# baler-collaboration/baler

Hardware: AMD Instinct MI355X
Metric: rows/sec (train) + rows/sec (encode), CMS 24-col AE at 1/2/4/8 GPUs (higher is better)
Workload: dtype f32

## Files before the change

baler_amd/csrc/fused.hip:

```cpp
#include "fused.hpp"

#include <cmath>
#include <cstdlib>
#include <type_traits>
#include <utility>

namespace bamd {
namespace {

using v4 = float __attribute__((ext_vector_type(4)));

__host__ __device__ constexpr int tiles(int d) { return (d + 15) / 16; }
__host__ __device__ constexpr int tile_steps(int d, int t) {
    return d - 16 * t >= 16 ? 4 : (d - 16 * t + 3) / 4;
}
__host__ __device__ constexpr int slot_feature(int d, int t, int g, int r) {
    int v = d - 16 * t;
    if (v >= 16) return 16 * t + 4 * g + r;
    return 4 * r + g < v ? 16 * t + 4 * r + g : -1;
}

constexpr int kQS = 68;
constexpr int kRowsPerWG = 64;

// ... 2094 lines not shown
        const bool v0 = r0 < n, v1 = r1 < n;
        constexpr int es = DZ16 ? 2 : 4;
        const __amdgpu_buffer_rsrc_t xrs = __builtin_amdgcn_make_buffer_rsrc((void *)((const char *)dz7 + (size_t)(grp * 128) * F * es), 0,
                                                                             0x7fffffff, 0x00020000);
        const int lr0 = wave * 32 + (lane & 15);
        const int xo0 = ((v0 ? lr0 : 0) * F + 8 * g) * es, xo1 = ((v1 ? lr0 + 16 : 0) * F + 8 * g) * es;
        asm volatile("" : "+v"(ws.voff), "+v"(w7.voff));
        v4 d6a[13], d6b[13];
        zero_tiles(d6a);
        zero_tiles(d6b);
        wide_in_product_bf16<F, DZ16>(d6a, d6b, wst, w7, xrs, xo0, xo1, wave, lane, g);
        auto narrow = [&](v4 (&d6)[13], int64_t row, bool valid) {
            const int64_t rrow = valid ? row : 0;
            Ring ring;
            ring_prime<S::total>(ring, ws);
            {
                v4 a[13];
                load_act<200>(a, y7, rrow, g);
                lrelu_bwd(d6, a);
            }
            store_rows<200>(d6, dz6, 0, row, valid, lane, nullptr, nullptr);
            v4 d5[7], d4[4], d3[tiles(Z)], d2[4], d1[7], d0[13];
            bwd_layer<N, S, 6>(d6, d5, ring, ws);
            { v4 a[7]; load_act<100>(a, y6, rrow, g); lrelu_bwd(d5, a); }
            store_rows<100>(d5, dz5, 0, row, valid, lane, nullptr, nullptr);
            bwd_layer<N, S, 5>(d5, d4, ring, ws);
            { v4 a[4]; load_act<50>(a, y5, rrow, g); lrelu_bwd(d4, a); }
            store_rows<50>(d4, dz4, 0, row, valid, lane, nullptr, nullptr);
            bwd_layer<N, S, 4>(d4, d3, ring, ws);
            if (dz_latent) {
                v4 e[tiles(Z)];
                load_act<Z>(e, dz_latent, rrow, g);
#pragma unroll
                for (int t = 0; t < tiles(Z); ++t) d3[t] += e[t];
            }
            store_rows<Z>(d3, dz3, 0, row, valid, lane, nullptr, nullptr);
            bwd_layer<N, S, 3>(d3, d2, ring, ws);
            { v4 a[4]; load_act<50>(a, y3, rrow, g); lrelu_bwd(d2, a); }
            store_rows<50>(d2, dz2, 0, row, valid, lane, nullptr, nullptr);
            bwd_layer<N, S, 2>(d2, d1, ring, ws);
            { v4 a[7]; load_act<100>(a, y2, rrow, g); lrelu_bwd(d1, a); }
            store_rows<100>(d1, dz1, 0, row, valid, lane, nullptr, nullptr);
            bwd_layer<N, S, 1>(d1, d0, ring, ws);
            { v4 a[13]; load_act<200>(a, y1, rrow, g); lrelu_bwd(d0, a); }
            store_rows<200>(d0, dz0, 0, row, valid, lane, nullptr, nullptr);
        };
        narrow(d6a, r0, v0);
        narrow(d6b, r1, v1);
    }
}

template <int NT>
__device__ __forceinline__ void q_write(float *__restrict__ q, const v4 (&a)[NT], int lane, int wave) {
    typedef float __attribute__((address_space(3))) *lds_f;
    const int col = 16 * wave + (lane & 15), g = lane >> 4;
#pragma unroll
    for (int r = 0; r < 4; ++r) {
        lds_f p = (lds_f)q + ((4 * g + r) * kQS + col);
        asm volatile("" : "+v"(p));
#pragma unroll
        for (int t = 0; t < NT; ++t) p[t * 16 * kQS] = a[t][r];
    }
}
template <int D>
__device__ __forceinline__ void q_write_x(float *__restrict__ q, const v4 (&a)[tiles(D)], int lane, int wave) {
    static_assert(D % 16 != 0, "ones slot lives in the partial last tile");
    constexpr int T = tiles(D) - 1, V = D - 16 * T;
    constexpr int R1 = V / 4, G1 = V % 4;
    typedef float __attribute__((address_space(3))) *lds_f;
    const int col = 16 * wave + (lane & 15), g = lane >> 4;
#pragma unroll
    for (int r = 0; r < 4; ++r) {
        lds_f p = (lds_f)q + ((4 * g + r) * kQS + col);
        asm volatile("" : "+v"(p));
#pragma unroll
        for (int t = 0; t < tiles(D); ++t) {
            float v = a[t][r];
            if (t == T && r == R1 && g == G1) v = 1.0f;
            p[t * 16 * kQS] = v;
        }
    }
}

template <class N, int l> struct DW {
    static constexpr int NT = tiles(N::dim(l + 1)), KT = tiles(N::dim(l) + 1), TOT = NT * KT, T = (TOT + 3) / 4;
    static constexpr int rows_x = 16 * KT, rows_dz = 16 * NT;
};

template <class N, int l>
__device__ __forceinline__ void dw_phase(const float *__restrict__ qdz, const float *__restrict__ qx,
                                         v4 (&acc)[DW<N, l>::T], int lane, int wave) {
    using D = DW<N, l>;
    constexpr int NP = (D::T + 1) / 2, U = 4 * NP;
    const int g = lane >> 4, i = lane & 15;
    typedef const float __attribute__((address_space(3))) *lds_cf;
    typedef const v4 __attribute__((address_space(3))) *lds_cv4;
    const lds_cf la = (lds_cf)qdz + (i * kQS + 4 * g), lb = (lds_cf)qx + (i * kQS + 4 * g);
    const lds_cf la_w = la + wave * (16 * kQS);
    v4 fa[2][2], fb[2][2];
    auto lds_frags = [&](int u, v4 (&a)[2], v4 (&b)[2]) {
#pragma unroll
        for (int h = 0; h < 2; ++h) {
            const int it = 2 * (u >> 2) + h;
            if (it < D::T) {
                const int c = (4 * it) % D::NT, k0 = (4 * it) / D::NT;
                if (c + 3 < D::NT && 4 * it + 3 < D::TOT) {
                    a[h] = *(lds_cv4)(la_w + c * (16 * kQS) + 16 * (u & 3));
                    b[h] = *(lds_cv4)(lb + k0 * (16 * kQS) + 16 * (u & 3));
                } else {
                    int idx = wave + 4 * it;
                    idx = idx < D::TOT ? idx : D::TOT - 1;
                    const int kt = idx / D::NT, nt = idx - kt * D::NT;
                    a[h] = *(lds_cv4)(la + nt * (16 * kQS) + 16 * (u & 3));
                    b[h] = *(lds_cv4)(lb + kt * (16 * kQS) + 16 * (u & 3));
                }
            }
        }
    };
    lds_frags(0, fa[0], fb[0]);
#pragma unroll
    for (int u = 0; u < U; ++u) {
        if (u + 1 < U) lds_frags(u + 1, fa[(u + 1) & 1], fb[(u + 1) & 1]);
        __builtin_amdgcn_sched_barrier(0);
        const int it0 = 2 * (u >> 2), it1 = it0 + 1;
#pragma unroll
        for (int r = 0; r < 4; ++r) {
            acc[it0] = mfma(fa[u & 1][0][r], fb[u & 1][0][r], acc[it0]);
            if (it1 < D::T) acc[it1] = mfma(fa[u & 1][1][r], fb[u & 1][1][r], acc[it1]);
        }
        __builtin_amdgcn_sched_barrier(0);
    }
}

template <class N, int l>
__device__ __forceinline__ void dw_flush(v4 *__restrict__ slab, const v4 (&acc)[DW<N, l>::T], int lane, int wave) {
#pragma unroll
    for (int it = 0; it < DW<N, l>::T; ++it) {
        const int idx = wave + 4 * it;
        if (idx < DW<N, l>::TOT) slab[(int64_t)(N::slab_off(l) + idx) * gridDim.x * 64 + lane] = acc[it];
    }
}

constexpr int kImgB = 320;
template <class N> constexpr int img_a_rows();
template <class N> constexpr bool train_bias_in_lds() {
    return (size_t)(img_a_rows<N>() + kImgB) * kQS * sizeof(float) + (size_t)(N::bf_off(8) - N::bf_off(0)) * 16 <= 160 * 1024;
}
template <class N> constexpr int img_a_rows() {
    int m = 240;
    const int need[] = {DW<N, 7>::rows_x + DW<N, 7>::rows_dz, DW<N, 5>::rows_x + DW<N, 5>::rows_dz, DW<N, 2>::rows_x + DW<N, 2>::rows_dz,
                        DW<N, 0>::rows_x + DW<N, 0>::rows_dz};
    for (int v : need) m = v > m ? v : m;
    return m;
}

template <int F, int Z, bool RT = false>
__global__ void __launch_bounds__(256) train_dec_kernel(const v4 *packed, const void *__restrict__ xin, int in_f64,
                                                        int64_t n, const double *__restrict__ feats, v4 *__restrict__ slabs,
                                                        v4 *__restrict__ dz_out, int fr, int zr) {
    using N = Net<F, Z>;
    using S = StreamTrainDec<N>;
    constexpr int kImgA = img_a_rows<N>();
    static_assert(DW<N, 7>::rows_x + DW<N, 7>::rows_dz <= kImgA && DW<N, 6>::rows_x + DW<N, 6>::rows_dz <= kImgB &&
                  DW<N, 5>::rows_x + DW<N, 5>::rows_dz <= kImgA && DW<N, 4>::rows_x + DW<N, 4>::rows_dz <= kImgB, "image buffers");
    extern __shared__ __attribute__((aligned(16))) float lds[];
    float *imgA = lds, *imgB = lds + kImgA * kQS;
// ... 165 lines not shown

        q_write_x<F>(imgA, a0, lane, wave); q_write(imgA + DW<N, 0>::rows_x * kQS, d1, lane, wave);
        __syncthreads();
        dw_phase<N, 0>(imgA + DW<N, 0>::rows_x * kQS, imgA, g0, lane, wave);
        ring_tail<S::total>(ring, ws);
    }
    dw_flush<N, 1>(slab, g1, lane, wave); dw_flush<N, 0>(slab, g0, lane, wave);
}
#else
template <int F, int Z, bool RT = false>
__global__ void __launch_bounds__(256) train_enc_kernel(const v4 *packed, const void *__restrict__ xin, int in_f64,
                                                        int64_t n, const double *__restrict__ feats, v4 *__restrict__ slabs,
                                                        const v4 *__restrict__ dz_in, int fr, int zr) {
    using N = Net<F, Z>;
    using S = StreamTrainEnc<N>;
    static_assert(Z <= 16, "dL/dz hand-off is one tile per row");
    constexpr int kImgA = img_a_rows<N>();
    static_assert(DW<N, 3>::rows_x + DW<N, 3>::rows_dz <= kImgB && DW<N, 2>::rows_x + DW<N, 2>::rows_dz <= kImgA &&
                  DW<N, 1>::rows_x + DW<N, 1>::rows_dz <= kImgB && DW<N, 0>::rows_x + DW<N, 0>::rows_dz <= kImgA, "image buffers");
    extern __shared__ __attribute__((aligned(16))) float lds[];
    float *imgA = lds, *imgB = lds + kImgA * kQS;
    const v4 *bias_lds = packed + N::bf_off(0);
    if constexpr (train_bias_in_lds<N>()) {
        v4 *stage = (v4 *)(lds + (kImgA + kImgB) * kQS);
        stage_bias<N>(stage, packed);
        bias_lds = stage;
    }
    int lane = threadIdx.x & 63, wave = __builtin_amdgcn_readfirstlane(threadIdx.x >> 6);
    v4 *slab = slabs + (int64_t)blockIdx.x * 64;
    const int64_t ngroups = (n + kRowsPerWG - 1) / kRowsPerWG;
    WStream ws = make_stream(packed + S::start_f4, (N::packed_f4() - S::start_f4) * 16, threadIdx.x & 63);
    v4 g3[DW<N, 3>::T], g2[DW<N, 2>::T], g1[DW<N, 1>::T], g0[DW<N, 0>::T];
    zero_tiles(g3); zero_tiles(g2); zero_tiles(g1); zero_tiles(g0);
    Ring ring;
    ring_prime<S::total>(ring, ws);
    v4 a0n[tiles(F)], d4n;
    {
        const int64_t row0 = (int64_t)blockIdx.x * kRowsPerWG + 16 * wave + (lane & 15);
        load_rows<F, RT>(a0n, xin, in_f64, row0, row0 < n, lane, feats, fr);
        d4n = row0 < n ? dz_in[row0 * 4 + (lane >> 4)] : (v4){0.f, 0.f, 0.f, 0.f};
    }
    for (int64_t grp = blockIdx.x; grp < ngroups; grp += gridDim.x) {
        asm volatile("" : "+v"(ws.voff), "+s"(wave), "+v"(lane));
        const int64_t row = grp * kRowsPerWG + 16 * wave + (lane & 15);
        const int64_t row_next = row + (int64_t)gridDim.x * kRowsPerWG;
        const bool valid_next = row_next < n;
        RawRows<F> xraw;
        v4 a0[tiles(F)], a1[13], a2[7], a3[4], d4[tiles(Z)];
#pragma unroll
        for (int t = 0; t < tiles(F); ++t) a0[t] = a0n[t];
        d4[0] = d4n;
        fwd_layer<N, S, 0>(a0, a1, ring, ws, bias_lds, lane);
        fwd_layer<N, S, 1>(a1, a2, ring, ws, bias_lds, lane);
        fwd_layer<N, S, 2>(a2, a3, ring, ws, bias_lds, lane);
        v4 d3[4], d2[7], d1[13];
        q_write_x<50>(imgB, a3, lane, wave); q_write(imgB + DW<N, 3>::rows_x * kQS, d4, lane, wave);
        bwd_layer<N, S, 3>(d4, d3, ring, ws); lrelu_bwd(d3, a3);
        __syncthreads();
        dw_phase<N, 3>(imgB + DW<N, 3>::rows_x * kQS, imgB, g3, lane, wave);

        q_write_x<100>(imgA, a2, lane, wave); q_write(imgA + DW<N, 2>::rows_x * kQS, d3, lane, wave);
        bwd_layer<N, S, 2>(d3, d2, ring, ws); lrelu_bwd(d2, a2);
        __syncthreads();
        dw_phase<N, 2>(imgA + DW<N, 2>::rows_x * kQS, imgA, g2, lane, wave);

        q_write_x<200>(imgB, a1, lane, wave); q_write(imgB + DW<N, 1>::rows_x * kQS, d2, lane, wave);
        bwd_layer<N, S, 1>(d2, d1, ring, ws); lrelu_bwd(d1, a1);
        __syncthreads();
        load_rows_issue<F, RT>(xraw, xin, in_f64, row_next, valid_next, lane, fr);
        v4 dzraw = valid_next ? dz_in[row_next * 4 + (lane >> 4)] : (v4){0.f, 0.f, 0.f, 0.f};
        dw_phase<N, 1>(imgB + DW<N, 1>::rows_x * kQS, imgB, g1, lane, wave);
        load_rows_finish<F, RT>(a0n, xraw, valid_next, lane, feats, fr);
        d4n = dzraw;

        q_write_x<F>(imgA, a0, lane, wave); q_write(imgA + DW<N, 0>::rows_x * kQS, d1, lane, wave);
        __syncthreads();
        dw_phase<N, 0>(imgA + DW<N, 0>::rows_x * kQS, imgA, g0, lane, wave);
        ring_tail<S::total>(ring, ws);
    }
    dw_flush<N, 3>(slab, g3, lane, wave); dw_flush<N, 2>(slab, g2, lane, wave);
    dw_flush<N, 1>(slab, g1, lane, wave); dw_flush<N, 0>(slab, g0, lane, wave);
}

#endif

template <class N> struct Lat {
    __host__ __device__ static constexpr int x_rows(int l) { return 16 * tiles(N::dim(l) + 1); }
    __host__ __device__ static constexpr int z_rows(int l) { return 16 * tiles(N::dim(l + 1)); }
    __host__ __device__ static constexpr int x_off(int l) { int s = 0; for (int j = 0; j < l; ++j) s += x_rows(j); return s; }
    __host__ __device__ static constexpr int z_off(int l) { int s = x_off(N::L); for (int j = 0; j < l; ++j) s += z_rows(j); return s; }
    static constexpr int xch_f4 = 13 * 64;
};


template <int NT> __device__ __forceinline__ void lat_collect(const v4 *xch, v4 (&all)[NT], int lane) {
#pragma unroll
    for (int t = 0; t < NT; ++t) all[t] = xch[t * 64 + lane];
}

constexpr int kImgStride = 16;

#ifdef BAMD_LAT_TRACE
__device__ unsigned long long g_lat_trace[64];
#define LAT_T(i) do { if (blockIdx.x == 0 && threadIdx.x == 0) g_lat_trace[i] = __builtin_amdgcn_s_memtime(); } while (0)
#else
#define LAT_T(i) do {} while (0)
#endif

template <class N, int W, int D_> struct LatSeq {
    static constexpr int D = D_, Wv = W, NG = 15;
    __host__ __device__ static constexpr int layer(int g) { return g < 8 ? g : 15 - g; }
    __host__ __device__ static constexpr int kd(int g) { return g < 8 ? N::dim(g) : N::dim(layer(g) + 1); }
    __host__ __device__ static constexpr int nt(int g) { return tiles(g < 8 ? N::dim(g + 1) : N::dim(layer(g))); }
    __host__ __device__ static constexpr int base(int g) { return (g < 8 ? N::wf_off(g) : N::wb_off(layer(g))) / 64; }
    __host__ __device__ static constexpr int nl(int g) { return (nt(g) + W - 1) / W; }
    __host__ __device__ static constexpr int nf(int g) { return tiles(kd(g)) * nl(g); }
    __host__ __device__ static constexpr int start(int g) { int s = 0; for (int j = 0; j < g; ++j) s += nf(j); return s; }
    static constexpr int total = start(NG);
    __host__ __device__ static constexpr int gemm_of(int G) { int g = 0; for (int j = 1; j < NG; ++j) if (G >= start(j)) g = j; return g; }
};
template <class SQ, int G>
__device__ __forceinline__ void seq_issue(v4 (&slot)[SQ::D], const WStream &ws, int wave) {
    if constexpr (G < SQ::total) {
        constexpr int g = SQ::gemm_of(G), f = G - SQ::start(g), NL = SQ::nl(g), q = f / NL, i = f % NL, NT = SQ::nt(g);
        int t = wave + SQ::Wv * i;
        t = t < NT ? t : NT - 1;
        slot[G % SQ::D] = frag_rt(ws, SQ::base(g) + q * NT + t);
    }
}
template <class SQ, int... G>
__device__ __forceinline__ void seq_prologue(v4 (&slot)[SQ::D], const WStream &ws, int wave, std::integer_sequence<int, G...>) {
    (seq_issue<SQ, G>(slot, ws, wave), ...);
    __builtin_amdgcn_sched_barrier(0);
}
template <class SQ, int g, int f>
__device__ __forceinline__ void seq_pair(const v4 (&in)[tiles(SQ::kd(g))], v4 (&out)[SQ::nl(g)], v4 (&slot)[SQ::D],
                                         const WStream &ws, int wave) {
    constexpr int NL = SQ::nl(g), NF = SQ::nf(g), S0 = SQ::start(g), KD = SQ::kd(g);
    constexpr bool two = f + 1 < NF;
    constexpr int q0 = f / NL, i0 = f % NL, q1 = two ? (f + 1) / NL : q0, i1 = two ? (f + 1) % NL : i0;
    constexpr int s0 = (S0 + f) % SQ::D, s1 = (S0 + f + (two ? 1 : 0)) % SQ::D;
#pragma unroll
    for (int r = 0; r < 4; ++r) {
        if (r < tile_steps(KD, q0)) out[i0] = mfma(slot[s0][r], in[q0][r], out[i0]);
        if (two && r < tile_steps(KD, q1)) out[i1] = mfma(slot[s1][r], in[q1][r], out[i1]);
    }
    seq_issue<SQ, S0 + f + SQ::D>(slot, ws, wave);
    if constexpr (two) seq_issue<SQ, S0 + f + 1 + SQ::D>(slot, ws, wave);
    __builtin_amdgcn_sched_barrier(0);
}
template <class SQ, int g, int... P>
__device__ __forceinline__ void seq_mm_impl(const v4 (&in)[tiles(SQ::kd(g))], v4 (&out)[SQ::nl(g)], v4 (&slot)[SQ::D],
                                            const WStream &ws, int wave, std::integer_sequence<int, P...>) {
    (seq_pair<SQ, g, 2 * P>(in, out, slot, ws, wave), ...);
}
template <class SQ, int g>
__device__ __forceinline__ void seq_mm(const v4 (&in)[tiles(SQ::kd(g))], v4 (&out)[SQ::nl(g)], v4 (&slot)[SQ::D], const WStream &ws,
                                       int wave) {
    seq_mm_impl<SQ, g>(in, out, slot, ws, wave, std::make_integer_sequence<int, (SQ::nf(g) + 1) / 2>{});
}
template <int D, bool ONES, int W>
__device__ __forceinline__ void lat2_publish(v4 *xch, __amdgpu_buffer_rsrc_t irs, int slot0, const v4 (&loc)[(tiles(D) + W - 1) / W],
                                             int lane, int wave) {
    constexpr int NT = tiles(D), NL = (NT + W - 1) / W;
    constexpr int T1 = tiles(D) - 1, V = D - 16 * T1, R1 = V / 4, G1 = V % 4;
    const int g = lane >> 4, col = lane & 15;
// ... 682 lines not shown
                        if (krow == ones_row) smap[b_off_r(l) + nf] = off;
                        else if (kt < tiles(K)) {
                            int kf = slot_feature(K, kt, j / 4, j % 4);
                            if (kf >= 0 && kf < Kr) smap[w_off_r(l) + nf * Kr + kf] = off;
                        }
                    }
    }
    for (int l = 0; l < kSplit - 1; ++l)
        for (int i = 0; i < N::wcount(l) * 4; ++i) src[(size_t)N::ef_off(l) * 4 + i] = src[(size_t)N::wf_off(l) * 4 + i];
    for (int l = kSplit - 1; l >= 1; --l)
        for (int i = 0; i < N::wcount(l) * 4; ++i) src[(size_t)N::eb_off(l) * 4 + i] = src[(size_t)N::wb_off(l) * 4 + i];
    bool exact = true;
    for (int i = 0; i <= N::L; ++i) exact = exact && h->dims[i] == N::dim(i);
    if (TRAIN && N::l4_frags() > 0 && exact) {
        for (int g = 0; g < 15; ++g) {
            const int l = g < 8 ? g : 15 - g, K = dim_r(l), NN = dim_r(l + 1);
            const int NO = N::l4_gemm_n(g);
            for (int k4 = 0; k4 < N::l4_ks(g); ++k4)
                for (int o = 0; o < NO; ++o)
                    for (int r = 0; r < 4; ++r) {
                        const int c = 4 * k4 + r;
                        const size_t at = ((size_t)N::l4_off() + N::l4_frag_off(g) + (size_t)k4 * NO + o) * 4 + r;
                        if (g < 8) { if (c < K) src[at] = w_off_r(l) + o * K + c; }
                        else if (c < NN) src[at] = w_off_r(l) + c * K + o;
                    }
        }
    }
    if (TRAIN) {
        for (int v : smap)
            if (v < 0) { set_error("fused: incomplete slab map"); return BAMD_ERR_INVALID; }
        std::vector<int> inv((size_t)N::slab_off(N::L) * 64 * 4, -1);
        for (int p = 0; p < nparams_r; ++p) inv[smap[p]] = p;
        smap.swap(inv);
    }
    {
        std::vector<int> off((size_t)nparams_r + 1, 0), idx;
        for (int v : src) if (v >= 0) off[v + 1]++;
        for (int p = 0; p < nparams_r; ++p) off[p + 1] += off[p];
        idx.resize(off[nparams_r]);
        std::vector<int> cur(off.begin(), off.end() - 1);
        for (size_t i = 0; i < src.size(); ++i) if (src[i] >= 0) idx[cur[src[i]]++] = (int)i;
        int rc2 = st->sc_off.ensure(off.size() * sizeof(int));
        if (rc2) return rc2;
        rc2 = st->sc_idx.ensure(idx.size() * sizeof(int));
        if (rc2) return rc2;
        BAMD_HIP(hipMemcpy(st->sc_off.p, off.data(), off.size() * sizeof(int), hipMemcpyHostToDevice));
        BAMD_HIP(hipMemcpy(st->sc_idx.p, idx.data(), idx.size() * sizeof(int), hipMemcpyHostToDevice));
    }
    st->packed_floats = (int)src.size();
    int rc = st->pack_src.ensure(src.size() * sizeof(int));
    if (rc) return rc;
    rc = st->slab_map.ensure(smap.size() * sizeof(int));
    if (rc) return rc;
    BAMD_HIP(hipMemcpy(st->pack_src.p, src.data(), src.size() * sizeof(int), hipMemcpyHostToDevice));
    BAMD_HIP(hipMemcpy(st->slab_map.p, smap.data(), smap.size() * sizeof(int), hipMemcpyHostToDevice));
    rc = h->packed.ensure(src.size() * sizeof(float));
    return rc;
}

constexpr int kBiasF4 = Net<24, 15>::bf_off(8) - Net<24, 15>::bf_off(0);

struct FusedOps {
    int (*setup)(bamd_handle *, FusedState *);
    int (*encode)(bamd_handle *, const void *, int, int64_t, const double *, void *, int, hipStream_t);
    int (*decode)(bamd_handle *, const void *, int, int64_t, const double *, const uint8_t *, void *, int, hipStream_t);
    int (*forward_loss)(bamd_handle *, const void *, int, int64_t, const double *, void *, int, double *, hipStream_t);
    int (*fwd_bwd)(bamd_handle *, const void *, int, int64_t, const double *, void *, hipStream_t);
    int (*train_step)(bamd_handle *, const void *, int, int64_t, const double *, void *, const AdamArgs &, hipStream_t);
    int (*wide_fwd)(bamd_handle *, const float *, int64_t, float *const *, float *, double *, int *, hipStream_t);
    int (*wide_bwd)(bamd_handle *, int64_t, float *const *, float *const *, const float *, hipStream_t);
    int (*pack_extra)(bamd_handle *, FusedState *, hipStream_t);
    bool throughput_training = true;
    bool (*wide_small)(const bamd_handle *, int64_t) = nullptr;
};

static FusedState *state_of(bamd_handle *h) { return (FusedState *)h->fused_state; }

static constexpr bool infer_pair() { return true; }
static int infer_grid(int64_t n) {
    int64_t wg = ((n + 15) / 16 + 3) / 4;
    return (int)(wg < 1 ? 1 : (wg > 1024 ? 1024 : wg));
}

template <int F, int Z, bool RT = false> struct Impl {
    using N = Net<F, Z>;
    static bool matches(const bamd_handle *h) {
        if (h->L != 8) return false;
        if (RT) {
            for (int i = 1; i <= 7; ++i)
                if (i != 4 && h->dims[i] != N::dim(i)) return false;
            return h->dims[0] == h->dims[8] && h->dims[0] >= 1 && h->dims[0] <= F && h->dims[4] >= 1 && h->dims[4] <= Z;
        }
        for (int i = 0; i <= 8; ++i)
            if (h->dims[i] != N::dim(i)) return false;
        return true;
    }
    static constexpr int train_lds = (img_a_rows<N>() + kImgB) * kQS * (int)sizeof(float) + (train_bias_in_lds<N>() ? (N::bf_off(8) - N::bf_off(0)) * 16 : 0);
    static int fr(const bamd_handle *h) { return h->dims[0]; }
    static int zr(const bamd_handle *h) { return h->dims[4]; }
    static int setup(bamd_handle *h, FusedState *st) {
        static_assert(RT || N::bf_off(8) - N::bf_off(0) == kBiasF4, "bias fragment count");
        static_assert(train_lds <= 160 * 1024, "LDS of the training pair");
        int rc = build_maps<F, Z, true>(h, st);
        if (rc) return rc;
        BAMD_HIP(hipFuncSetAttribute((const void *)train_dec_kernel<F, Z, RT>, hipFuncAttributeMaxDynamicSharedMemorySize, train_lds));
        BAMD_HIP(hipFuncSetAttribute((const void *)train_enc_kernel<F, Z, RT>, hipFuncAttributeMaxDynamicSharedMemorySize, train_lds));
        return BAMD_OK;
    }
    static int encode(bamd_handle *h, const void *x, int x_dtype, int64_t n, const double *features, void *z, int z_dtype,
                      hipStream_t s) {
        constexpr int extra_lds = 0;
        if (F <= 64 && infer_pair()) {
            hipLaunchKernelGGL((infer2_kernel<F <= 64 ? F : 24, Z, K_ENCODE, RT>), dim3(infer_grid((n + 1) / 2)), dim3(256), 0, s,
                               (const v4 *)h->packed.p, x, x_dtype == BAMD_F64, n, features, z, z_dtype,
                               (const uint8_t *)nullptr, fr(h), zr(h));
            BAMD_HIP(hipGetLastError());
            return BAMD_OK;
        }
        hipLaunchKernelGGL((infer_kernel<F, Z, K_ENCODE, RT>), dim3(infer_grid(n)), dim3(256), extra_lds, s, (const v4 *)h->packed.p, x,
                           x_dtype == BAMD_F64, n, features, z, z_dtype, (const uint8_t *)nullptr, (double *)nullptr, fr(h), zr(h));
        BAMD_HIP(hipGetLastError());
        return BAMD_OK;
    }
    static int decode(bamd_handle *h, const void *z, int z_dtype, int64_t n, const double *features, const uint8_t *int_mask,
                      void *out, int out_dtype, hipStream_t s) {
        if (F <= 64 && infer_pair()) {
            hipLaunchKernelGGL((infer2_kernel<F <= 64 ? F : 24, Z, K_DECODE, RT>), dim3(infer_grid((n + 1) / 2)), dim3(256), 0, s,
                               (const v4 *)h->packed.p, z, z_dtype, n, features, out, out_dtype == BAMD_F64, int_mask, fr(h), zr(h));
            BAMD_HIP(hipGetLastError());
            return BAMD_OK;
        }
        hipLaunchKernelGGL((infer_kernel<F, Z, K_DECODE, RT>), dim3(infer_grid(n)), dim3(256), 0, s, (const v4 *)h->packed.p, z,
                           z_dtype, n, features, out, out_dtype == BAMD_F64, int_mask, (double *)nullptr, fr(h), zr(h));
        BAMD_HIP(hipGetLastError());
        return BAMD_OK;
    }
    static int forward_loss(bamd_handle *h, const void *x, int x_dtype, int64_t n, const double *features, void *recon,
                            int recon_dtype, double *loss_sum, hipStream_t s) {
        int grid = infer_grid(n);
        int rc = h->lossp.ensure(sizeof(double) * 1024);
        if (rc) return rc;
        hipLaunchKernelGGL((infer_kernel<F, Z, K_FORWARD, RT>), dim3(grid), dim3(256), 0, s, (const v4 *)h->packed.p, x,
                           x_dtype == BAMD_F64, n, features, recon, recon_dtype == BAMD_F64, (const uint8_t *)nullptr,
                           (double *)h->lossp.p, fr(h), zr(h));
        hipLaunchKernelGGL(sum_partials_fixed_k<double>, dim3(1), dim3(256), 0, s, (const double *)h->lossp.p, grid, 1.0 / fr(h), loss_sum, 0);
        BAMD_HIP(hipGetLastError());
        return BAMD_OK;
    }
    static int fwd_bwd(bamd_handle *h, const void *x, int x_dtype, int64_t n, const double *features, void *grads,
                       hipStream_t s) {
        FusedState *st = state_of(h);
        const int np = (int)h->nparams;
        if (n <= st->latency_max_rows) return small_batch(h, x, x_dtype, n, features, grads, nullptr, s);
        int64_t ngroups = (n + kRowsPerWG - 1) / kRowsPerWG;
        int grid = (int)(ngroups < st->nwg_max ? ngroups : st->nwg_max);
        int64_t tail_rows = 0;
        if (ngroups > grid && ngroups % grid != 0 && ngroups % grid <= 32 && st->tail_split) {
            const int64_t main_rows = (ngroups - ngroups % grid) * kRowsPerWG;
            tail_rows = n - main_rows;
            n = main_rows;
            ngroups -= ngroups % grid;
        }
        int rc = h->slabs.ensure((size_t)N::slab_f4() * 16 * (size_t)grid);
        if (rc) return rc;
        rc = st->dz.ensure((size_t)(ngroups + grid) * kRowsPerWG * (kSplit == 2 ? 7 * 64 : 64));
        if (rc) return rc;
        hipLaunchKernelGGL((train_dec_kernel<F, Z, RT>), dim3(grid), dim3(256), train_lds, s, (const v4 *)h->packed.p, x,
                           x_dtype == BAMD_F64, n, features, (v4 *)h->slabs.p, (v4 *)st->dz.p, fr(h), zr(h));
        hipLaunchKernelGGL((train_enc_kernel<F, Z, RT>), dim3(grid), dim3(256), train_lds, s, (const v4 *)h->packed.p, x,
                           x_dtype == BAMD_F64, n, features, (v4 *)h->slabs.p, (const v4 *)st->dz.p, fr(h), zr(h));
        hipLaunchKernelGGL(reduce_slabs_k<float>, dim3(N::slab_off(N::L) + 1), dim3(256), 0, s, (const v4 *)h->slabs.p, grid,
                           N::slab_off(N::L), (const int *)st->slab_map.p, np, 1.0 / fr(h), (float *)grads);
        BAMD_HIP(hipGetLastError());
        if (tail_rows > 0) {
            const char *xt = (const char *)x + (size_t)n * fr(h) * dtype_bytes(x_dtype);
            return small_batch(h, xt, x_dtype, tail_rows, features, grads, nullptr, s, true);
        }
        return BAMD_OK;
    }
    static int small_batch(bamd_handle *h, const void *x, int x_dtype, int64_t n, const double *features, void *grads,
                           const AdamArgs *ad, hipStream_t s, bool accumulate = false) {
        FusedState *st = state_of(h);
        const int nblk = (int)((n + 15) / 16);
        constexpr size_t img_bytes = (size_t)Lat<N>::z_off(N::L) * kImgStride * sizeof(float);
        int rc = st->imgs.ensure(img_bytes * (size_t)nblk);
        if (rc) return rc;
        rc = h->lossp.ensure(sizeof(double) * (size_t)(4 * nblk > 1024 ? 4 * nblk : 1024));
        if (rc) return rc;
        int nloss = nblk;
        bool four_row = false;
        if constexpr (!RT) {
            if (n <= st->lat4_max_rows) {
                four_row = true;
                nloss = 4 * nblk;
                hipLaunchKernelGGL((lat4_chain_kernel<F, Z, RT>), dim3(4 * nblk), dim3(256), 0, s, (const v4 *)h->packed.p + N::l4_off(),
                                   (const float *)h->params.p, x, x_dtype == BAMD_F64, n, features, (float *)st->imgs.p, (double *)h->lossp.p,
                                   fr(h), zr(h));
            }
        }
        if (!four_row)
            hipLaunchKernelGGL((lat2_chain_kernel<F, Z, 4, RT>), dim3(nblk), dim3(256), 0, s, (const v4 *)h->packed.p, x,
                               x_dtype == BAMD_F64, n, features, (float *)st->imgs.p, (double *)h->lossp.p, fr(h), zr(h));
        const dim3 grid(8 * ((N::slab_off(N::L) + 1 + 7) / 8));
        const int nsplit = nblk >= 512 ? 4 : 1;
        float *part = nullptr;
        if (nsplit > 1) {
            rc = st->dwpart.ensure((size_t)(N::slab_off(N::L) + 1) * nsplit * 256 * sizeof(float));
            if (rc) return rc;
            part = (float *)st->dwpart.p;
        }
        auto launch = [&](auto mode, const AdamArgs &aa) {
            constexpr int M = decltype(mode)::value;
            if (nsplit > 1) {
                hipLaunchKernelGGL((lat2_dw_kernel<N, M>), dim3(grid.x, nsplit), dim3(256), 0, s, (const float *)st->imgs.p, nblk,
                                   (const double *)h->lossp.p, nloss, (const int *)st->slab_map.p, (float *)grads, aa, part, nsplit, 1, (int)h->nparams, 1.0 / fr(h));
                hipLaunchKernelGGL((lat2_dw_kernel<N, M>), grid, dim3(256), 0, s, (const float *)st->imgs.p, nblk,
                                   (const double *)h->lossp.p, nloss, (const int *)st->slab_map.p, (float *)grads, aa, part, nsplit, 2, (int)h->nparams, 1.0 / fr(h));
            } else
                hipLaunchKernelGGL((lat2_dw_kernel<N, M>), grid, dim3(256), 0, s, (const float *)st->imgs.p, nblk,
                                   (const double *)h->lossp.p, nloss, (const int *)st->slab_map.p, (float *)grads, aa, part, 1, 0, (int)h->nparams, 1.0 / fr(h));
        };
        if (ad) launch(std::integral_constant<int, DW_ADAM>{}, *ad);
        else if (accumulate) launch(std::integral_constant<int, DW_ACCUM>{}, AdamArgs{});
        else launch(std::integral_constant<int, DW_WRITE>{}, AdamArgs{});
        BAMD_HIP(hipGetLastError());
        return BAMD_OK;
    }
    static int train_step(bamd_handle *h, const void *x, int x_dtype, int64_t n, const double *features, void *grads,
                          const AdamArgs &ad, hipStream_t s) {
        FusedState *st = state_of(h);
        if (n > st->latency_max_rows) return BAMD_ERR_UNSUPPORTED;
        return small_batch(h, x, x_dtype, n, features, grads, &ad, s);
    }
    static const FusedOps *ops() {
        static const FusedOps o = {setup, encode, decode, forward_loss, fwd_bwd, train_step};
        return &o;
    }
};

template <int F, int Z, bool SMALL = true> struct ImplInferClass {
    using B = Impl<F, Z, true>;
    static_assert(F % 16 == 15 && Z % 16 == 15 && (F <= 127 || !SMALL), "class widths are 16 T - 1; the small-batch chain takes up to 8 input tiles");
    static bool matches(const bamd_handle *h) { return B::matches(h); }
    static int setup(bamd_handle *h, FusedState *st) { return build_maps<F, Z, SMALL>(h, st); }
    static int fwd_bwd(bamd_handle *h, const void *x, int x_dtype, int64_t n, const double *features, void *grads, hipStream_t s) {
        if constexpr (SMALL) {
            if (n <= state_of(h)->latency_max_rows) return B::small_batch(h, x, x_dtype, n, features, grads, nullptr, s);
            const char *ce = getenv("BALER_AMD_CLASS_CHUNK_ROWS");
            const int64_t chunk = ce ? atoll(ce) : 65536;
            if (chunk >= 16) {
                const size_t row_bytes = (size_t)B::fr(h) * dtype_bytes(x_dtype);
                const int64_t ck = chunk & ~(int64_t)15;
                for (int64_t r0 = 0; r0 < n; r0 += ck) {
// ... 762 lines not shown
```

Baseline: 298.4 million.

## Split training kernels into producer and weight-gradient consumer wave roles

```diff
diff --git a/baler_amd/csrc/fused.hip b/baler_amd/csrc/fused.hip
--- a/baler_amd/csrc/fused.hip
+++ b/baler_amd/csrc/fused.hip
@@ -2200,6 +2200,30 @@
     }
 }
 
+template <int D>
+__device__ __forceinline__ void lrelu_bwd_img(v4 (&d)[tiles(D)], const float *__restrict__ q, int lane, int wave) {
+    constexpr int T = tiles(D) - 1, V = D - 16 * T, R1 = V / 4, G1 = V % 4;
+    typedef const float __attribute__((address_space(3))) *lds_cf;
+    const int col = 16 * wave + (lane & 15), g = lane >> 4;
+    lds_cf p[4];
+#pragma unroll
+    for (int r = 0; r < 4; ++r) {
+        p[r] = (lds_cf)q + ((4 * g + r) * kQS + col);
+        asm volatile("" : "+v"(p[r]));
+    }
+#pragma unroll
+    for (int t = 0; t < tiles(D); ++t) {
+        v4 sl;
+#pragma unroll
+        for (int r = 0; r < 4; ++r) {
+            float y = p[r][t * 16 * kQS];
+            if (t == T && r == R1) y = g == G1 ? 0.f : y;
+            sl[r] = y > 0.f ? 1.0f : 0.01f;
+        }
+        d[t] = d[t] * sl;
+    }
+}
+
 template <class N, int l> struct DW {
     static constexpr int NT = tiles(N::dim(l + 1)), KT = tiles(N::dim(l) + 1), TOT = NT * KT, T = (TOT + 3) / 4;
     static constexpr int rows_x = 16 * KT, rows_dz = 16 * NT;
@@ -2531,6 +2555,197 @@
     dw_flush<N, 1>(slab, g1, lane, wave); dw_flush<N, 0>(slab, g0, lane, wave);
 }
 
+#endif
+
+#if BAMD_SPLIT == 2
+template <int F, int Z, bool RT = false>
+__global__ void __launch_bounds__(512) train_dec_roles_kernel(const v4 *packed, const void *__restrict__ xin, int in_f64,
+                                                              int64_t n, const double *__restrict__ feats, v4 *__restrict__ slabs,
+                                                              v4 *__restrict__ dz_out, int fr, int zr) {
+    using N = Net<F, Z>;
+    using S = StreamTrainDec<N>;
+    constexpr int kImgA = img_a_rows<N>();
+    static_assert(DW<N, 7>::rows_x + DW<N, 7>::rows_dz <= kImgA && DW<N, 6>::rows_x + DW<N, 6>::rows_dz <= kImgB &&
+                  DW<N, 5>::rows_x + DW<N, 5>::rows_dz <= kImgA && DW<N, 4>::rows_x + DW<N, 4>::rows_dz <= kImgB &&
+                  DW<N, 3>::rows_x + DW<N, 3>::rows_dz <= kImgA && DW<N, 2>::rows_x + DW<N, 2>::rows_dz <= kImgB, "image buffers");
+    extern __shared__ __attribute__((aligned(16))) float lds[];
+    float *imgA = lds, *imgB = lds + kImgA * kQS;
+    const v4 *bias_lds = packed + N::bf_off(0);
+    if constexpr (train_bias_in_lds<N>()) {
+        v4 *stage = (v4 *)(lds + (kImgA + kImgB) * kQS);
+        stage_bias<N>(stage, packed);
+        bias_lds = stage;
+    }
+    int lane = threadIdx.x & 63, wave = __builtin_amdgcn_readfirstlane(threadIdx.x >> 6);
+    const int64_t ngroups = (n + kRowsPerWG - 1) / kRowsPerWG;
+    double lacc = 0.0;
+    if (wave >= 4) {
+        int tw = wave - 4;
+        v4 *slab = slabs + (int64_t)blockIdx.x * 64;
+        v4 g7[DW<N, 7>::T], g6[DW<N, 6>::T], g5[DW<N, 5>::T], g4[DW<N, 4>::T], g3[DW<N, 3>::T], g2[DW<N, 2>::T];
+        zero_tiles(g7); zero_tiles(g6); zero_tiles(g5); zero_tiles(g4); zero_tiles(g3); zero_tiles(g2);
+        for (int64_t grp = blockIdx.x; grp < ngroups; grp += gridDim.x) {
+            asm volatile("" : "+s"(tw), "+v"(lane));
+            __syncthreads();
+            dw_phase<N, 7>(imgA + DW<N, 7>::rows_x * kQS, imgA, g7, lane, tw);
+            __syncthreads();
+            dw_phase<N, 6>(imgB + DW<N, 6>::rows_x * kQS, imgB, g6, lane, tw);
+            __syncthreads();
+            dw_phase<N, 5>(imgA + DW<N, 5>::rows_x * kQS, imgA, g5, lane, tw);
+            __syncthreads();
+            dw_phase<N, 4>(imgB + DW<N, 4>::rows_x * kQS, imgB, g4, lane, tw);
+            __syncthreads();
+            dw_phase<N, 3>(imgA + DW<N, 3>::rows_x * kQS, imgA, g3, lane, tw);
+            __syncthreads();
+            dw_phase<N, 2>(imgB + DW<N, 2>::rows_x * kQS, imgB, g2, lane, tw);
+        }
+        dw_flush<N, 7>(slab, g7, lane, tw); dw_flush<N, 6>(slab, g6, lane, tw);
+        dw_flush<N, 5>(slab, g5, lane, tw); dw_flush<N, 4>(slab, g4, lane, tw);
+        dw_flush<N, 3>(slab, g3, lane, tw); dw_flush<N, 2>(slab, g2, lane, tw);
+    } else {
+        WStream ws = make_stream(packed + S::start_f4, (N::packed_f4() - S::start_f4) * 16, lane);
+        Ring ring;
+        ring_prime<S::total>(ring, ws);
+        v4 a0n[tiles(F)];
+        {
+            const int64_t row0 = (int64_t)blockIdx.x * kRowsPerWG + 16 * wave + (lane & 15);
+            load_rows<F, RT>(a0n, xin, in_f64, row0, row0 < n, lane, feats, fr);
+        }
+        for (int64_t grp = blockIdx.x; grp < ngroups; grp += gridDim.x) {
+            asm volatile("" : "+v"(ws.voff), "+s"(wave), "+v"(lane));
+            const int64_t row = grp * kRowsPerWG + 16 * wave + (lane & 15);
+            const bool valid = row < n;
+            const int64_t row_next = row + (int64_t)gridDim.x * kRowsPerWG;
+            const bool valid_next = row_next < n;
+            RawRows<F> xraw;
+            v4 a2[7], a3[4], a4[tiles(Z)], a5[4], a6[7], a7[13], d8[tiles(F)];
+            {
+                v4 a0[tiles(F)], a1[13];
+#pragma unroll
+                for (int t = 0; t < tiles(F); ++t) a0[t] = a0n[t];
+                fwd_layer<N, S, 0>(a0, a1, ring, ws, bias_lds, lane);
+                fwd_layer<N, S, 1>(a1, a2, ring, ws, bias_lds, lane);
+                fwd_layer<N, S, 2>(a2, a3, ring, ws, bias_lds, lane);
+                fwd_layer<N, S, 3>(a3, a4, ring, ws, bias_lds, lane);
+                fwd_layer<N, S, 4>(a4, a5, ring, ws, bias_lds, lane);
+                fwd_layer<N, S, 5>(a5, a6, ring, ws, bias_lds, lane);
+                fwd_layer<N, S, 6>(a6, a7, ring, ws, bias_lds, lane);
+                fwd_layer<N, S, 7>(a7, d8, ring, ws, bias_lds, lane);
+#pragma unroll
+                for (int t = 0; t < tiles(F); ++t)
+#pragma unroll
+                    for (int r = 0; r < 4; ++r) {
+                        float d = d8[t][r] - a0[t][r];
+                        const bool live = valid && slot_feature(F, t, lane >> 4, r) >= 0;
+                        if (live) lacc += (double)d * (double)d;
+                        d8[t][r] = live ? d * (2.0f / (float)(RT ? fr : F)) : 0.f;
+                    }
+            }
+            v4 d7[13], d6[7], d5[4], d4[tiles(Z)], d3[4], d2[7];
+            q_write_x<200>(imgA, a7, lane, wave); q_write(imgA + DW<N, 7>::rows_x * kQS, d8, lane, wave);
+            bwd_layer<N, S, 7>(d8, d7, ring, ws); lrelu_bwd_img<200>(d7, imgA, lane, wave);
+            __syncthreads();
+
+            q_write_x<100>(imgB, a6, lane, wave); q_write(imgB + DW<N, 6>::rows_x * kQS, d7, lane, wave);
+            bwd_layer<N, S, 6>(d7, d6, ring, ws); lrelu_bwd(d6, a6);
+            __syncthreads();
+            load_rows_issue<F, RT>(xraw, xin, in_f64, row_next, valid_next, lane, fr);
+
+            q_write_x<50>(imgA, a5, lane, wave); q_write(imgA + DW<N, 5>::rows_x * kQS, d6, lane, wave);
+            bwd_layer<N, S, 5>(d6, d5, ring, ws); lrelu_bwd(d5, a5);
+            __syncthreads();
+            load_rows_finish<F, RT>(a0n, xraw, valid_next, lane, feats, fr);
+
+            q_write_x<Z>(imgB, a4, lane, wave); q_write(imgB + DW<N, 4>::rows_x * kQS, d5, lane, wave);
+            bwd_layer<N, S, 4>(d5, d4, ring, ws);
+            __syncthreads();
+
+            q_write_x<50>(imgA, a3, lane, wave); q_write(imgA + DW<N, 3>::rows_x * kQS, d4, lane, wave);
+            bwd_layer<N, S, 3>(d4, d3, ring, ws); lrelu_bwd(d3, a3);
+            __syncthreads();
+
+            q_write_x<100>(imgB, a2, lane, wave); q_write(imgB + DW<N, 2>::rows_x * kQS, d3, lane, wave);
+            bwd_layer<N, S, 2>(d3, d2, ring, ws); lrelu_bwd(d2, a2);
+#pragma unroll
+            for (int t = 0; t < 7; ++t) dz_out[((row >> 4) * 7 + t) * 64 + lane] = d2[t];
+            __syncthreads();
+            ring_tail<S::total>(ring, ws);
+        }
+    }
+    __syncthreads();
+    const double wsum = block_sum_tree(lacc, (double *)lds);
+    if (threadIdx.x == 0) ((double *)(slabs + (int64_t)N::slab_off(N::L) * gridDim.x * 64))[blockIdx.x] = wsum;
+}
+
+template <int F, int Z, bool RT = false>
+__global__ void __launch_bounds__(512) train_enc_roles_kernel(const v4 *packed, const void *__restrict__ xin, int in_f64,
+                                                              int64_t n, const double *__restrict__ feats, v4 *__restrict__ slabs,
+                                                              const v4 *__restrict__ dz_in, int fr, int zr) {
+    using N = Net<F, Z>;
+    using S = StreamTrainEnc<N>;
+    constexpr int kImgA = img_a_rows<N>();
+    static_assert(DW<N, 1>::rows_x + DW<N, 1>::rows_dz <= kImgB && DW<N, 0>::rows_x + DW<N, 0>::rows_dz <= kImgA, "image buffers");
+    extern __shared__ __attribute__((aligned(16))) float lds[];
+    float *imgA = lds, *imgB = lds + kImgA * kQS;
+    const v4 *bias_lds = packed + N::bf_off(0);
+    if constexpr (train_bias_in_lds<N>()) {
+        v4 *stage = (v4 *)(lds + (kImgA + kImgB) * kQS);
+        stage_bias<N>(stage, packed);
+        bias_lds = stage;
+    }
+    int lane = threadIdx.x & 63, wave = __builtin_amdgcn_readfirstlane(threadIdx.x >> 6);
+    const int64_t ngroups = (n + kRowsPerWG - 1) / kRowsPerWG;
+    if (wave >= 4) {
+        int tw = wave - 4;
+        v4 *slab = slabs + (int64_t)blockIdx.x * 64;
+        v4 g1[DW<N, 1>::T], g0[DW<N, 0>::T];
+        zero_tiles(g1); zero_tiles(g0);
+        for (int64_t grp = blockIdx.x; grp < ngroups; grp += gridDim.x) {
+            asm volatile("" : "+s"(tw), "+v"(lane));
+            __syncthreads();
+            dw_phase<N, 1>(imgB + DW<N, 1>::rows_x * kQS, imgB, g1, lane, tw);
+            __syncthreads();
+            dw_phase<N, 0>(imgA + DW<N, 0>::rows_x * kQS, imgA, g0, lane, tw);
+        }
+        dw_flush<N, 1>(slab, g1, lane, tw); dw_flush<N, 0>(slab, g0, lane, tw);
+    } else {
+        WStream ws = make_stream(packed + S::start_f4, (N::packed_f4() - S::start_f4) * 16, lane);
+        Ring ring;
+        ring_prime<S::total>(ring, ws);
+        v4 a0n[tiles(F)], d2n[7];
+        {
+            const int64_t row0 = (int64_t)blockIdx.x * kRowsPerWG + 16 * wave + (lane & 15);
+            load_rows<F, RT>(a0n, xin, in_f64, row0, row0 < n, lane, feats, fr);
+#pragma unroll
+            for (int t = 0; t < 7; ++t) d2n[t] = dz_in[((row0 >> 4) * 7 + t) * 64 + lane];
+        }
+        for (int64_t grp = blockIdx.x; grp < ngroups; grp += gridDim.x) {
+            asm volatile("" : "+v"(ws.voff), "+s"(wave), "+v"(lane));
+            const int64_t row = grp * kRowsPerWG + 16 * wave + (lane & 15);
+            const int64_t row_next = row + (int64_t)gridDim.x * kRowsPerWG;
+            const bool valid_next = row_next < n;
+            RawRows<F> xraw;
+            v4 a0[tiles(F)], a1[13], d2[7], d1[13];
+#pragma unroll
+            for (int t = 0; t < tiles(F); ++t) a0[t] = a0n[t];
+#pragma unroll
+            for (int t = 0; t < 7; ++t) d2[t] = d2n[t];
+            fwd_layer<N, S, 0>(a0, a1, ring, ws, bias_lds, lane);
+
+            q_write_x<200>(imgB, a1, lane, wave); q_write(imgB + DW<N, 1>::rows_x * kQS, d2, lane, wave);
+            bwd_layer<N, S, 1>(d2, d1, ring, ws); lrelu_bwd(d1, a1);
+            __syncthreads();
+            load_rows_issue<F, RT>(xraw, xin, in_f64, row_next, valid_next, lane, fr);
+#pragma unroll
+            for (int t = 0; t < 7; ++t) d2n[t] = dz_in[((row_next >> 4) * 7 + t) * 64 + lane];
+
+            q_write_x<F>(imgA, a0, lane, wave); q_write(imgA + DW<N, 0>::rows_x * kQS, d1, lane, wave);
+            __syncthreads();
+            load_rows_finish<F, RT>(a0n, xraw, valid_next, lane, feats, fr);
+            ring_tail<S::total>(ring, ws);
+        }
+    }
+}
 #endif
 
 template <class N> struct Lat {
@@ -3379,6 +3594,8 @@
     return (int)(wg < 1 ? 1 : (wg > 1024 ? 1024 : wg));
 }
 
+constexpr int kTrainRolesDefault = 1;
+
 template <int F, int Z, bool RT = false> struct Impl {
     using N = Net<F, Z>;
     static bool matches(const bamd_handle *h) {
@@ -3393,6 +3610,7 @@
         return true;
     }
     static constexpr int train_lds = (img_a_rows<N>() + kImgB) * kQS * (int)sizeof(float) + (train_bias_in_lds<N>() ? (N::bf_off(8) - N::bf_off(0)) * 16 : 0);
+    static constexpr bool train_roles = kSplit == 2 && !RT && tiles(F) <= 2;
     static int fr(const bamd_handle *h) { return h->dims[0]; }
     static int zr(const bamd_handle *h) { return h->dims[4]; }
     static int setup(bamd_handle *h, FusedState *st) {
@@ -3402,6 +3620,10 @@
         if (rc) return rc;
         BAMD_HIP(hipFuncSetAttribute((const void *)train_dec_kernel<F, Z, RT>, hipFuncAttributeMaxDynamicSharedMemorySize, train_lds));
         BAMD_HIP(hipFuncSetAttribute((const void *)train_enc_kernel<F, Z, RT>, hipFuncAttributeMaxDynamicSharedMemorySize, train_lds));
+        if constexpr (train_roles) {
+            BAMD_HIP(hipFuncSetAttribute((const void *)train_dec_roles_kernel<F, Z, RT>, hipFuncAttributeMaxDynamicSharedMemorySize, train_lds));
+            BAMD_HIP(hipFuncSetAttribute((const void *)train_enc_roles_kernel<F, Z, RT>, hipFuncAttributeMaxDynamicSharedMemorySize, train_lds));
+        }
         return BAMD_OK;
     }
     static int encode(bamd_handle *h, const void *x, int x_dtype, int64_t n, const double *features, void *z, int z_dtype,
@@ -3462,10 +3684,21 @@
         if (rc) return rc;
         rc = st->dz.ensure((size_t)(ngroups + grid) * kRowsPerWG * (kSplit == 2 ? 7 * 64 : 64));
         if (rc) return rc;
-        hipLaunchKernelGGL((train_dec_kernel<F, Z, RT>), dim3(grid), dim3(256), train_lds, s, (const v4 *)h->packed.p, x,
-                           x_dtype == BAMD_F64, n, features, (v4 *)h->slabs.p, (v4 *)st->dz.p, fr(h), zr(h));
-        hipLaunchKernelGGL((train_enc_kernel<F, Z, RT>), dim3(grid), dim3(256), train_lds, s, (const v4 *)h->packed.p, x,
-                           x_dtype == BAMD_F64, n, features, (v4 *)h->slabs.p, (const v4 *)st->dz.p, fr(h), zr(h));
+        bool roles = false;
+        if constexpr (train_roles) roles = env_ll("BALER_AMD_TRAIN_ROLES", kTrainRolesDefault) != 0;
+        if (roles) {
+            if constexpr (train_roles) {
+                hipLaunchKernelGGL((train_dec_roles_kernel<F, Z, RT>), dim3(grid), dim3(512), train_lds, s, (const v4 *)h->packed.p, x,
+                                   x_dtype == BAMD_F64, n, features, (v4 *)h->slabs.p, (v4 *)st->dz.p, fr(h), zr(h));
+                hipLaunchKernelGGL((train_enc_roles_kernel<F, Z, RT>), dim3(grid), dim3(512), train_lds, s, (const v4 *)h->packed.p, x,
+                                   x_dtype == BAMD_F64, n, features, (v4 *)h->slabs.p, (const v4 *)st->dz.p, fr(h), zr(h));
+            }
+        } else {
+            hipLaunchKernelGGL((train_dec_kernel<F, Z, RT>), dim3(grid), dim3(256), train_lds, s, (const v4 *)h->packed.p, x,
+                               x_dtype == BAMD_F64, n, features, (v4 *)h->slabs.p, (v4 *)st->dz.p, fr(h), zr(h));
+            hipLaunchKernelGGL((train_enc_kernel<F, Z, RT>), dim3(grid), dim3(256), train_lds, s, (const v4 *)h->packed.p, x,
+                               x_dtype == BAMD_F64, n, features, (v4 *)h->slabs.p, (const v4 *)st->dz.p, fr(h), zr(h));
+        }
         hipLaunchKernelGGL(reduce_slabs_k<float>, dim3(N::slab_off(N::L) + 1), dim3(256), 0, s, (const v4 *)h->slabs.p, grid,
                            N::slab_off(N::L), (const int *)st->slab_map.p, np, 1.0 / fr(h), (float *)grads);
         BAMD_HIP(hipGetLastError());
```

After: 303.2 million, median of 6. 1.02x the previous value.
